# l90lpa/fv3-jedi-linearmodel

Hardware: AMD Instinct MI355X
Metric: column-updates/s per TL+AD dyn step (higher is better)
Workload: dtype f64; 1 GPU; C192L127 hydrostatic TL+AD, six cube faces dealt over 1 GPU(s) (6 per rank), table-driven exchange (221184 columns per GPU), k_split=2 n_split=6 dt=450s nq=4, hord mt/vt/tm/dp/tr=2/2/2/2/2 (sponge: 1/1/1/1 below level 9), kord=17, nord=1; columns_per_gpu=221184

## Files before the change

### fv3_jedi_linearmodel_amd/csrc/dycore.h

```cpp
#pragma once
#include "../../include/fv3lm.h"
#include "stages.h"
#include "column.h"
#include "exchange.h"
#include "nh.h"
#include "nh_ad.h"
#include "tpfused.h"
#include "tpad.h"
#include "tp2.h"
#include "dampt.h"
#include <functional>
#include <map>
#include <memory>
#include <set>
#include <string>
#include <vector>

namespace fv3 {

#ifdef FV3LM_HOST_EMUL
inline void* dev_alloc(size_t n) { void* p = std::calloc(n ? n : 1, 1); return p; }
inline void dev_free(void* p) { std::free(p); }
inline void dev_zero(Exec&, void* p, size_t n) { std::memset(p, 0, n); }
inline void dev_copy(Exec&, void* d, const void* s, size_t n) { std::memcpy(d, s, n); }
// ... 42 lines not shown
    Fld f; f.t = t + used; f.p = p + used; f.nk = nk; used += n; return f;
  }
};

struct CkSet {
  struct Item { std::string name; double* p; size_t n, off; };
  std::string name; std::vector<Item> items; size_t stride = 0; int nrec = 0; double* buf = nullptr;
  void add(const std::string& nm, double* p, size_t ndoubles) { items.push_back(Item{nm, p, ndoubles, stride}); stride += ndoubles; }
  void add(const std::string& nm, const Fld& f, size_t plane) { add(nm, f.t, (size_t)f.nk * plane); }
  void alloc(const char* nm, int nrec_) {
    name = nm; buf = nrec_ > 0 ? (double*)dev_alloc(stride * nrec_ * 8) : nullptr; nrec = buf ? nrec_ : 0;
    if (std::getenv("FV3LM_VERBOSE")) std::fprintf(stderr, "fv3lm: checkpoint set %s: %d records, %zu bytes\n", nm, nrec, stride * nrec * 8);
  }
  void destroy() { dev_free(buf); buf = nullptr; nrec = 0; }
  int item(const char* nm) const {
    for (int n = 0; n < (int)items.size(); ++n) if (items[(size_t)n].name == nm) return n;
    set_sticky("internal error: checkpoint set " + name + " has no item " + nm); return -1;
  }
  size_t bytes(int item) const { return items[(size_t)item].n * 8; }
  double* at(int rec, int item) const {
    if (buf && rec >= 0 && rec < nrec && item >= 0 && item < (int)items.size()) return buf + (size_t)rec * stride + items[(size_t)item].off;
    set_sticky("internal error: checkpoint set " + name + ": record " + std::to_string(rec) + " item " + std::to_string(item) + " out of range"); return nullptr;
  }
  void save(Exec& ex, int rec, int item) const { if (double* q_ = at(rec, item)) dev_copy(ex, q_, items[(size_t)item].p, bytes(item)); }
  void restore(Exec& ex, int rec, int item, double* to = nullptr) const {
    if (const double* q_ = at(rec, item)) dev_copy(ex, to ? to : items[(size_t)item].p, q_, bytes(item));
  }
  void save(Exec& ex, int rec) const { for (int n = 0; n < (int)items.size(); ++n) save(ex, rec, n); }
  void restore(Exec& ex, int rec) const { for (int n = 0; n < (int)items.size(); ++n) restore(ex, rec, n); }
  void redirect(Exec& ex, int rec, int item, const double* from) const { if (double* q_ = at(rec, item)) ex.redirect_t(from, q_); }
};

typedef fv3lm_options Options;

inline bool resolve_level(const Options& o, int k, int npz, LevelParams& lp) {
  int hord_m = o.hord_mt, hord_t = o.hord_tm, hord_v = o.hord_vt, hord_p = o.hord_dp;
  int nord_k = o.nord, nord_v = (2 > o.nord) ? o.nord : 2;
  double d2_divg = (0.20 > o.d2_bg) ? o.d2_bg : 0.20;
  double damp_vt = o.do_vort_damp ? o.vtdm4 : 0.;
  int nord_w = nord_v, nord_t = nord_v;
  double damp_w = damp_vt, damp_t = damp_vt, d_con_k = o.d_con;
  if (npz == 1 || o.n_sponge < 0) {
    d2_divg = o.d2_bg;
  } else if (k == 1) {
    nord_k = 0;
    if (0.01 < o.d2_bg) d2_divg = (o.d2_bg < o.d2_bg_k1) ? o.d2_bg_k1 : o.d2_bg;
    else if (0.01 < o.d2_bg_k1) d2_divg = o.d2_bg_k1;
    else d2_divg = 0.01;
    nord_w = 0; damp_w = d2_divg;
    if (o.do_vort_damp) { nord_v = 0; damp_vt = 0.5 * d2_divg; }
    d_con_k = 0.;
  } else {
    const int max1 = (2 < o.n_sponge - 1) ? o.n_sponge - 1 : 2;
    if (k == max1 && o.d2_bg_k2 > 0.01) {
      nord_k = 0; d2_divg = (o.d2_bg < o.d2_bg_k2) ? o.d2_bg_k2 : o.d2_bg;
      nord_w = 0; damp_w = d2_divg;
      if (o.do_vort_damp) { nord_v = 0; damp_vt = 0.5 * d2_divg; }
      d_con_k = 0.;
    } else {
      const int max2 = (3 < o.n_sponge) ? o.n_sponge : 3;
      if (k == max2 && o.d2_bg_k2 > 0.05) {
        nord_k = 0; d2_divg = (o.d2_bg < 0.2 * o.d2_bg_k2) ? 0.2 * o.d2_bg_k2 : o.d2_bg;
        nord_w = 0; damp_w = d2_divg; d_con_k = 0.;
      }
    }
  }
// ... 98 lines not shown
  bool reuse_fields = false;
  Fld S(const char* n, int nk) {
    if (reuse_fields) { auto it = F.find(n); if (it != F.end()) return it->second; }
    (nk == g.npz ? nS3 : nS3p)++; Fld x = state.take((size_t)ntile_all * nk * g.plane, nk); F[n] = x; return x; }
  int nW3 = 0, nW3p = 0, nS3 = 0, nS3p = 0;
  Fld W(const char* n, int nk) {
    if (reuse_fields) { auto it = F.find(n); if (it != F.end()) return it->second; }
    (nk == g.npz ? nW3 : nW3p)++; Fld x = work.take((size_t)ntile_all * nk * g.plane, nk); F[n] = x; return x; }

  Rect R(int i0, int i1, int j0, int j1) const { return Rect{i0, i1, j0, j1}; }
  static Rect empty_in(const Rect& r) { return Rect{r.i0 + 1, r.i0, r.j0 + 1, r.j0}; }
  static Rect isect(const Rect& a, const Rect& b) { return Rect{std::max(a.i0, b.i0), std::min(a.i1, b.i1), std::max(a.j0, b.j0), std::min(a.j1, b.j1)}; }
  static bool is_empty(const Rect& r) { return r.i0 > r.i1 || r.j0 > r.j1; }
  template <class D>
  void add_face(Program& P, const char* grp, const D& s, int W) {
    if (!g.face) { add(P, grp, Edged<D, false>(s)); return; }
    const int lo = 1 + W, hi = g.nx - W, BIG = 1 << 20;
    const Rect regs[5] = {{lo, hi, lo, hi}, {-BIG, BIG, -BIG, lo - 1}, {-BIG, BIG, hi + 1, BIG}, {-BIG, lo - 1, lo, hi}, {hi + 1, BIG, lo, hi}};
    std::vector<Edged<D, true>> strips; bool have_bulk = false; Edged<D, false> bulk;
    for (int r = 0; r < 5; ++r) {
      D t = s; Rect anchor{1, 0, 1, 0}; bool any = false;
      for (int n = 0; n < D::NOUT; ++n) {
        t.orect[n] = isect(s.orect[n], regs[r]);
        if (!is_empty(t.orect[n]) && !any) { anchor = t.orect[n]; any = true; }
      }
      if (!any) continue;
      for (int n = 0; n < D::NOUT; ++n) if (is_empty(t.orect[n])) t.orect[n] = empty_in(anchor);
      if (r == 0) {
        for (int m = 0; m < D::NIN; ++m) if ((edge_only_inputs((const D*)nullptr) >> m) & 1u) { const int nk = t.in[m].nk; t.in[m] = Fld{}; t.in[m].nk = nk; }
        bulk = Edged<D, false>(t); have_bulk = true;
      } else strips.push_back(Edged<D, true>(t));
    }
    const size_t n0 = P.size();
    add_multi(P, grp, strips);
    const size_t n1 = P.size();
    if (have_bulk) add(P, grp, bulk);
#ifndef FV3LM_HOST_EMUL
    if (have_bulk && n1 == n0 + 1 && P.size() == n1 + 1) {
      auto fs = P[n0].fn; auto fb = P[n1].fn;
      P[n0].fn = [fs](Exec& e, int mode) {
        if (mode == MODE_AD || !e.sstream) { fs(e, mode); return; }
        HIPCHK(hipEventRecord(e.ev_s0, e.stream)); HIPCHK(hipStreamWaitEvent(e.sstream, e.ev_s0, 0));
        hipStream_t main = e.stream; e.stream = e.sstream;
        fs(e, mode);
        e.stream = main;
        HIPCHK(hipEventRecord(e.ev_s1, e.sstream)); e.side_pending = true;
      };
      P[n1].fn = [fb](Exec& e, int mode) {
        fb(e, mode);
        if (e.side_pending) { HIPCHK(hipStreamWaitEvent(e.stream, e.ev_s1, 0)); e.side_pending = false; }
      };
    }
#endif
  }

  template <class St>
  static void declare(Op& op, const St& s) {
    for (int m = 0; m < St::NIN; ++m) if (St::wants(m) && s.in[m].p) { op.ad_in.push_back(s.in[m].p); op.ad_in_slot.push_back(m); }
    for (int n = 0; n < St::NOUT; ++n) { op.ad_out.push_back(s.out[n].p); op.ad_out_rect.push_back(s.orect[n]); }
  }
  template <class St>
  void add(Program& P, const char* group, const St& s) {
    Ctx* cp = &ctx;
    auto sp = std::make_shared<St>(s);
    Op op{group, [sp, cp](Exec& e, int mode) { run(e, mode, *sp, *cp); }};
    declare(op, s);
    op.set_wmask = [sp](unsigned w, Rect r) { sp->wmask = w; sp->wrect = r; };
    op.name = St::name();
    P.push_back(op);
  }
  template <class St>
  void add_multi(Program& P, const char* group, const std::vector<St>& v) {
    if (v.empty()) return;
    if (v.size() == 1) { add(P, group, v[0]); return; }
    Ctx* cp = &ctx;
    Op op{group, [v, cp](Exec& e, int mode) { run_multi(e, mode, v.data(), (int)v.size(), *cp); }};
    for (const St& s : v) declare(op, s);
    op.ad_in_slot.clear();
    op.name = St::name();
    P.push_back(op);
  }
  void halo(int mode, int kind, const Fld& f0, const Fld& f1 = Fld{}) {
    if (!g.face) { run_halo(ex, mode, g, f0); if (f1.t) run_halo(ex, mode, g, f1); return; }
    if (xt[kind].n == 0 && !xr[kind].active) { halo_missing = true; return; }
    run_exchange(ex, mode, g, xt[kind], ex.sh(f0), ex.sh(f1));
    if (!run_exchange_remote(ex, mode, g, xr[kind], ex.sh(f0), ex.sh(f1), err)) halo_missing = true;
  }
  void add_halo(Program& P, const char* group, int kind, Fld f0, Fld f1 = Fld{}, int when = 0) {
    Dycore* self = this;
    Op op{group, [self, kind, f0, f1, when](Exec&, int mode) {
      if (self->g.face && ((when == 1 && self->last_acoustic) || (when == 2 && !self->last_acoustic))) return;
      if (!self->g.face && when == 2) return;
      self->halo(mode, kind, f0, f1);
    }};
    op.ad_in = {f0.p, f1.p};
    op.name = "halo"; op.global = true;
    P.push_back(op);
  }
  void halo_window(int mode, bool start, int win, int kind, const Fld& f0, const Fld& f1) {
#ifndef FV3LM_HOST_EMUL
    if (ex.xstream) {
      if (start) {
        HIPCHK(hipEventRecord(ex.ev_a[win], ex.stream)); HIPCHK(hipStreamWaitEvent(ex.xstream, ex.ev_a[win], 0));
        hipStream_t main = ex.stream; ex.stream = ex.xstream;
        halo(mode, kind, f0, f1);
        ex.stream = main;
        HIPCHK(hipEventRecord(ex.ev_b[win], ex.xstream));
      } else HIPCHK(hipStreamWaitEvent(ex.stream, ex.ev_b[win], 0));
      return;
    }
#endif
    (void)win;
    if (!start) halo(mode, kind, f0, f1);
// ... 199 lines not shown
        }
        Op ad{grp, [a, cp, adf](Exec& e, int) { if (adf == 2) run_tp_ad(e, a, *cp); else run_tp_outer_ad(e, a, *cp); }};
        ad.modes = 1u << MODE_AD; ad.name = adf == 2 ? "TpAd" : "TpOuter";
        ad.ad_out = {fx.p, fy.p}; ad.ad_out_rect = {R(is, ie + 1, js, je), R(is, ie, js, je + 1)};
        if (adf == 2) ad.ad_in = {q.p, crx.p, cry.p, xfx.p, yfx.p, rax.p, ray.p, mx.p, my.p};
        else { ad.ad_store = {q_i.p, q_j.p, fx2.p, fy2.p}; ad.ad_in = {crx.p, cry.p, mx.p, my.p}; }
        P.push_back(ad);
      }
    }
  }
  void build_a2b(Program& P, const char* grp, const std::string& pre, Fld q, Fld qb, int nk) {
    const int is = g.is(), ie = g.ie(), js = g.js(), je = g.je();
    Fld qx = W((pre + "_qx").c_str(), nk), qy = W((pre + "_qy").c_str(), nk);
    const int npx = g.nx + 1, npy = g.ny + 1;
    A2bA_<false> a; a.in[0] = q; a.out[0] = qx; a.out[1] = qy; a.k1 = nk;
    A2bB_<false> b; b.in[0] = qx; b.in[1] = qy; b.in[2] = Fld{}; b.out[0] = qb; b.k1 = nk;
    if (!g.face) {
      a.orect[0] = R(is, ie + 1, js - 2, je + 2); a.orect[1] = R(is - 2, ie + 2, js, je + 1); add(P, grp, a);
      b.orect[0] = R(is, ie + 1, js, je + 1); add(P, grp, b);
      return;
    }
    const Rect qxr = R(is, ie + 1, std::max(1, js - 2), std::min(npy - 1, je + 2)), qyr = R(std::max(1, is - 2), std::min(npx - 1, ie + 2), js, je + 1);
    a.orect[0] = isect(qxr, R(3, npx - 2, qxr.j0, qxr.j1)); a.orect[1] = isect(qyr, R(qyr.i0, qyr.i1, 3, npy - 2));
    const bool a0 = !is_empty(a.orect[0]), a1 = !is_empty(a.orect[1]);
    if (a0 && !a1) a.orect[1] = empty_in(a.orect[0]);
    if (a1 && !a0) a.orect[0] = empty_in(a.orect[1]);
    A2bA_<true> ae; ae.in[0] = q; ae.out[0] = qx; ae.out[1] = qy; ae.k1 = nk;
    std::vector<A2bA_<true>> av;
    for (int e = 0; e < 4; ++e) {
      const Rect r = e == 0 ? isect(qxr, R(1, 2, qxr.j0, qxr.j1)) : e == 1 ? isect(qxr, R(npx - 1, npx, qxr.j0, qxr.j1)) : e == 2 ? isect(qyr, R(qyr.i0, qyr.i1, 1, 2)) : isect(qyr, R(qyr.i0, qyr.i1, npy - 1, npy));
      if (is_empty(r)) continue;
      ae.orect[e < 2 ? 0 : 1] = r; ae.orect[e < 2 ? 1 : 0] = empty_in(r); av.push_back(ae);
    }
    add_multi(P, grp, av);
    if (a0 || a1) add(P, grp, a);
    const Rect qbr = R(is, ie + 1, js, je + 1);
    b.orect[0] = isect(qbr, R(3, npx - 2, 3, npy - 2));
    A2bB_<true> be; be.in[0] = qx; be.in[1] = qy; be.in[2] = q; be.out[0] = qb; be.k1 = nk;
    std::vector<A2bB_<true>> bv;
    for (int e = 0; e < 4; ++e) {
      const Rect r = isect(qbr, e == 0 ? R(1, npx, 1, 2) : e == 1 ? R(1, npx, npy - 1, npy) : e == 2 ? R(1, 2, 3, npy - 2) : R(npx - 1, npx, 3, npy - 2));
      if (is_empty(r)) continue;
      be.orect[0] = r; bv.push_back(be);
    }
    add_multi(P, grp, bv);
    if (!is_empty(b.orect[0])) add(P, grp, b);
  }

  void build_acoustic();
  bool init(int nx, int ny, int npz, int ntile, int face, int nq_, double bdt_, int n_split_, int k_split_, const Options& o,
            const double* const* metrics_host, double da_min, double da_min_c, const double* phis_host, int nface = 0, const int* ij0 = nullptr);
  void destroy();

  void run_group(Progs& P, const char* group, int mode, bool skip_accum = false);
  void zero_work_adjoint() { dev_zero(ex, work.p, work.used * 8); }
  void dyn_core(int mode);
};

inline void Dycore::run_group(Progs& PS, const char* group, int mode, bool skip_accum) {
  const bool all = (group == nullptr) || (group[0] == 0);
  ex.skip_accum = skip_accum;
  const int nc = (int)PS.c.size();
  auto take = [&](const Op& op) { return (all || op.group == group) && !(mode != MODE_AD && skip_accum && op.accum) && ((op.modes >> mode) & 1u); };
  if (nc == 1) {
    set_class(0);
    const Program& P = PS.c[0];
    if (mode != MODE_AD) { for (const Op& op : P) if (take(op)) { if (op.global) set_class(-1); op.fn(ex, mode); if (op.global) set_class(0); } }
    else for (auto it = P.rbegin(); it != P.rend(); ++it) if (take(*it)) { if (it->global) set_class(-1); it->fn(ex, mode); if (it->global) set_class(0); }
    set_class(-1);
    ex.skip_accum = false;
    return;
  }
  std::vector<std::vector<size_t>> gl(nc);
  for (int c = 0; c < nc; ++c) for (size_t n = 0; n < PS.c[c].size(); ++n) if (PS.c[c][n].global) gl[c].push_back(n);
  for (int c = 1; c < nc; ++c) if (gl[c].size() != gl[0].size()) { set_sticky("internal error: the tile classes' programs hold different exchange sequences"); ex.skip_accum = false; return; }
  const size_t nseg = gl[0].size() + 1;
  auto seg = [&](int c, size_t sg, size_t& a, size_t& b) { a = sg == 0 ? 0 : gl[c][sg - 1] + 1; b = sg < gl[c].size() ? gl[c][sg] : PS.c[c].size(); };
  if (mode != MODE_AD) {
    for (size_t sg = 0; sg < nseg; ++sg) {
// ... 70 lines not shown
  if (!nh && npz < 2) { err = "hydrostatic vertical remap: the column map (edge values of cs_profile / scalar_profile) needs npz >= 2"; return false; }
  if (nh && !(o.a_imp > 0.5)) { err = "non-hydrostatic: a_imp must be > 0.5 (semi-implicit solver; the reference's a_imp <= 0.5 Riemann-invariant solver is not built)"; return false; }
  for (int kd : {o.kord_tm_pert, o.kord_mt_pert, o.kord_wz_pert, o.kord_tr_pert})
    if ((kd < 0 ? -kd : kd) <= 16) { err = "kord_*_pert: only |kord| > 16 (the linear profile, the one the TL/AD reference differentiates) is built"; return false; }
  for (int kd : {o.kord_tm, o.kord_mt, o.kord_wz, o.kord_tr}) {
    const int ak = kd < 0 ? -kd : kd;
    if (ak <= 16 && !(ak >= 8 && ak <= 15)) { err = "kord_tm/kord_mt/kord_wz/kord_tr: the linear profile (|kord| > 16) or, for the trajectory, the limited profiles 8 .. 15 of cs_profile / scalar_profile (not 16, not ppm_profile's 7 and below)"; return false; }
    if (ak <= 16 && npz < 6) { err = "kord: limited trajectory profiles need npz >= 6"; return false; }
  }
  lev_host.resize(npz + 1);
  for (int k = 1; k <= npz; ++k) {
    resolve_level(o, k, npz, lev_host[k - 1]);
    const LevelParams& l = lev_host[k - 1];
    for (int h : {l.hord_mt, l.hord_vt, l.hord_tm, l.hord_dp, l.hord_tr, l.hord_tm_g})
      if (h != 1 && h != 2 && h != 333) { err = "perturbation hord must be 1, 2 or 333 (the schemes the TL/AD reference implements)"; return false; }
    for (int h : {l.hord_mt_t, l.hord_vt_t, l.hord_tm_t, l.hord_dp_t, l.hord_tr_t, l.hord_tm_g_t})
      if (h != 333 && !(h >= 1 && h <= 13)) { err = "trajectory hord must be 1, 2, 333 (differentiated) or, with a different perturbation scheme, 3 .. 13"; return false; }
    const int pairs[6][2] = {{l.hord_mt_t, l.hord_mt}, {l.hord_vt_t, l.hord_vt}, {l.hord_tm_t, l.hord_tm}, {l.hord_dp_t, l.hord_dp}, {l.hord_tr_t, l.hord_tr}, {l.hord_tm_g_t, l.hord_tm_g}};
    for (auto& pr : pairs) if (pr[0] == pr[1] && pr[0] != 1 && pr[0] != 2 && pr[0] != 333) { err = "hord must be 1, 2 or 333 where trajectory and perturbation share the scheme"; return false; }
  }
#ifndef FV3LM_HOST_EMUL
  HIPCHK(hipStreamCreate(&ex.stream));
  { const char* env = std::getenv("FV3LM_NO_ASYNC_HALO");
    if (face && !(env && env[0] == '1')) {
      HIPCHK(hipStreamCreate(&ex.xstream));
      for (int w = 0; w < Exec::NWIN; ++w) { HIPCHK(hipEventCreateWithFlags(&ex.ev_a[w], hipEventDisableTiming)); HIPCHK(hipEventCreateWithFlags(&ex.ev_b[w], hipEventDisableTiming)); }
    }
    const char* es = std::getenv("FV3LM_NO_SIDE_STRIPS");
    if (face && !(es && es[0] == '1')) {
      HIPCHK(hipStreamCreate(&ex.sstream));
      HIPCHK(hipEventCreateWithFlags(&ex.ev_s0, hipEventDisableTiming)); HIPCHK(hipEventCreateWithFlags(&ex.ev_s1, hipEventDisableTiming));
    } }
#endif
  lev_host[npz] = lev_host[npz - 1];
  lev_dev = (LevelParams*)dev_alloc(sizeof(LevelParams) * (npz + 1));
  h2d(ex, lev_dev, lev_host.data(), sizeof(LevelParams) * (npz + 1));
  const size_t np = (size_t)ntile * g.plane;
  metric_dev.resize(NMETRIC);
  for (int m = 0; m < NMETRIC; ++m) { metric_dev[m] = (double*)dev_alloc(np * 8); h2d(ex, metric_dev[m], metrics_host[m], np * 8); }
  Metrics& M = ctx.m; int m = 0;
  const double** slots[] = {&M.area, &M.rarea, &M.rarea_c, &M.dx, &M.dy, &M.dxa, &M.dya, &M.dxc, &M.dyc, &M.rdx, &M.rdy, &M.rdxa,
                            &M.rdya, &M.rdxc, &M.rdyc, &M.cosa, &M.sina, &M.rsina, &M.cosa_u, &M.cosa_v, &M.cosa_s, &M.sina_u,
                            &M.sina_v, &M.rsin_u, &M.rsin_v, &M.rsin2, &M.f0, &M.fC, &M.del6_u, &M.del6_v, &M.divg_u, &M.divg_v};
  for (auto s : slots) *s = metric_dev[m++];
  M.sin_sg[0] = M.cos_sg[0] = nullptr;
  for (int n = 1; n <= 9; ++n) M.sin_sg[n] = metric_dev[m++];
  for (int n = 1; n <= 9; ++n) M.cos_sg[n] = metric_dev[m++];
  M.da_min = da_min; M.da_min_c = da_min_c;
  edge_dev = (double*)dev_alloc((size_t)ntile * 4 * g.pj * 8); ecorner_dev = (double*)dev_alloc((size_t)ntile * 12 * 8);
  M.edge = edge_dev; M.ecorner = ecorner_dev;
  m_all = M;
  hs_dev = (double*)dev_alloc(np * 8);
  if (phis_host) h2d(ex, hs_dev, phis_host, np * 8);
  ctx.g = g; ctx.lev = lev_dev; ctx.nlev = npz;
  n3 = np * npz; n3p = np * (npz + 1);
  state.init(n3 * (12 + (size_t)nq + (nh ? 5 + (size_t)nq : 0)) + n3p * (6 + (nh ? 2 : 0)) + np);
  if (nh) {
    nh_ws = (double*)dev_alloc((size_t)NH_WS_SLOTS * (npz + 2) * np * 8);
    const char* tape_env = std::getenv("FV3LM_NH_TAPE");
    const bool tape_on = tape_env && tape_env[0] == '1';
    nh_tape.cap = tape_on ? 104 * (npz + 2) : 1;
    int tape_tiles = tape_on ? ntile : 1;
    if (tape_on) {
#ifndef FV3LM_HOST_EMUL
    { size_t fr = 0, tot = 0;
      if (hipMemGetInfo(&fr, &tot) != hipSuccess) fr = 0;
// ... 170 lines not shown
    for (const char* n_ : {"w", "delz", "zh"}) st_in.push_back(n_);
    for (const char* n_ : {"w_o", "delz_o", "zh_o"}) st_out.push_back(n_);
  }
  Fld utmp = W("utmp", npz), vtmp = W("vtmp", npz), ua = W("ua", npz), va = W("va", npz);
  { CswInterpAD s; s.in[0] = u; s.in[1] = v; s.out[0] = utmp; s.out[1] = vtmp; s.out[2] = ua; s.out[3] = va;
    s.orect[0] = R(isd, ied, js - 1, je + 1); s.orect[1] = R(is - 1, ie + 1, jsd, jed);
    s.orect[2] = s.orect[3] = R(is - 1, ie + 1, js - 1, je + 1);
    if (g.face) {
      const int il = is == 1 ? isd : is - 1, ih = ie == g.nx ? ied : ie + 1, jl = js == 1 ? jsd : js - 1, jh = je == g.ny ? jed : je + 1;
      s.orect[0] = R(isd, ied, jl, jh); s.orect[1] = R(il, ih, jsd, jed); s.orect[2] = s.orect[3] = R(il, ih, jl, jh);
    }
    s.k1 = npz; add_face(P, "c_sw", s, 3); }
  Fld uc0 = W("uc0", npz), utf = W("utf", npz), vc0 = W("vc0", npz), vtf = W("vtf", npz);
  const Fld none{};
  { CswInterpC_<false> s; s.in[0] = utmp; s.in[1] = vtmp; s.in[2] = u; s.in[3] = v; s.out[0] = uc0; s.out[1] = utf; s.out[2] = vc0; s.out[3] = vtf;
    s.dt2 = dt2; s.k1 = npz;
    if (!g.face) {
      s.orect[0] = s.orect[1] = R(is - 1, ie + 2, js - 1, je + 1); s.orect[2] = s.orect[3] = R(is - 1, ie + 1, js - 1, je + 2); add(P, "c_sw", s);
    } else {
      const int npx = g.nx + 1, npy = g.ny + 1;
      const Rect ur = R(is - 1, ie + 2, js - 1, je + 1), vr = R(is - 1, ie + 1, js - 1, je + 2);
      s.orect[0] = s.orect[1] = isect(ur, R(3, npx - 2, ur.j0, ur.j1)); s.orect[2] = s.orect[3] = isect(vr, R(vr.i0, vr.i1, 3, npy - 2));
      const bool b0 = !is_empty(s.orect[0]), b2 = !is_empty(s.orect[2]);
      if (b0 && !b2) s.orect[2] = s.orect[3] = empty_in(s.orect[0]);
      if (b2 && !b0) s.orect[0] = s.orect[1] = empty_in(s.orect[2]);
      CswInterpC_<true> e; for (int n = 0; n < 4; ++n) { e.in[n] = s.in[n]; e.out[n] = s.out[n]; }
      e.in[4] = ua; e.in[5] = va; e.dt2 = dt2; e.k1 = npz;
      std::vector<CswInterpC_<true>> ev;
      for (int m = 0; m < 4; ++m) {
        const Rect r = m == 0 ? isect(ur, R(ur.i0, 2, ur.j0, ur.j1)) : m == 1 ? isect(ur, R(npx - 1, ur.i1, ur.j0, ur.j1)) : m == 2 ? isect(vr, R(vr.i0, vr.i1, vr.j0, 2)) : isect(vr, R(vr.i0, vr.i1, npy - 1, vr.j1));
        if (is_empty(r)) continue;
        e.orect[0] = e.orect[1] = m < 2 ? r : empty_in(r); e.orect[2] = e.orect[3] = m < 2 ? empty_in(r) : r; ev.push_back(e);
      }
      add_multi(P, "c_sw", ev);
      if (b0 || b2) add(P, "c_sw", s);
    } }
  Fld divgd = W("divgd", npz);
  if (opt.nord > 0) {
    CswDivgD s; s.in[0] = u; s.in[1] = v; s.in[2] = ua; s.in[3] = va; s.out[0] = divgd; s.orect[0] = R(is, ie + 1, js, je + 1); s.k1 = npz;
    add_face(P, "c_sw", s, 1);
  }
  Fld delpc = W("delpc", npz), ptc = W("ptc", npz);
  { CswTransportD s; s.in[0] = delp; s.in[1] = pt; s.in[2] = utf; s.in[3] = vtf; s.out[0] = delpc; s.out[1] = ptc;
    s.orect[0] = s.orect[1] = R(is - 1, ie + 1, js - 1, je + 1); s.k1 = npz; add_face(P, "c_sw", s, 1); }
  Fld wc{};
  if (nh) {
    wc = W("wc", npz);
    CswTransportWD s; s.in[0] = delp; s.in[1] = w; s.in[2] = utf; s.in[3] = vtf; s.in[4] = delpc; s.out[0] = wc;
    s.orect[0] = R(is - 1, ie + 1, js - 1, je + 1); s.k1 = npz; add_face(P, "c_sw", s, 1);
  }
  Fld ke_c = W("ke_c", npz), vort_c = W("vort_c", npz);
  { CswKeVortD s; s.in[0] = ua; s.in[1] = va; s.in[2] = uc0; s.in[3] = vc0; s.in[4] = g.face ? u : none; s.in[5] = g.face ? v : none; s.out[0] = ke_c; s.out[1] = vort_c;
    s.orect[0] = R(is - 1, ie + 1, js - 1, je + 1); s.orect[1] = R(is, ie + 1, js, je + 1); s.dt2 = dt2; s.k1 = npz; add_face(P, "c_sw", s, 1); }
  Fld uc1 = W("uc1", npz), vc1 = W("vc1", npz);
  { CswUpdateD s; s.in[0] = uc0; s.in[1] = vc0; s.in[2] = u; s.in[3] = v; s.in[4] = vort_c; s.in[5] = ke_c; s.out[0] = uc1; s.out[1] = vc1;
    s.orect[0] = R(is, ie + 1, js, je); s.orect[1] = R(is, ie, js, je + 1); s.dt2 = dt2; s.k1 = npz; add_face(P, "c_sw", s, 1); }
  Fld pe_c = W("pe_c", npz + 1), peln_c = W("peln_c", npz + 1), pkc = W("pkc", npz + 1), gz = W("gz", npz + 1);
  Fld uc = W("uc", npz), vc = W("vc", npz);
  if (nh) {
    Fld gz_a = W("gz_a", npz + 1);
    Fld xfz = W("xfz", npz + 1), yfz = W("yfz", npz + 1);
    { DzFluxC s; s.in[0] = utf; s.in[1] = vtf; s.out[0] = xfz; s.out[1] = yfz; s.orect[0] = R(is - 1, ie + 2, js - 1, je + 1);
      s.orect[1] = R(is - 1, ie + 1, js - 1, je + 2); s.k1 = npz + 1; add(P, "update_dz_c", s); }
    { UpdateDzCD s; s.in[0] = zh; s.in[1] = xfz; s.in[2] = yfz; s.out[0] = gz_a; s.orect[0] = R(is - 1, ie + 1, js - 1, je + 1); s.k1 = npz + 1;
      add_face(P, "update_dz_c", s, 1); }
    { NhColArgs a = nh_args(dt2); a.f[0] = gz_a; a.f[1] = wc; a.f[2] = ptc; a.f[3] = delpc; a.f[4] = gz; a.f[5] = pkc;
      add_col(P, "riem_c", NHC_RIEM_C, a, R(is - 1, ie + 1, js - 1, je + 1)); }
    PGradCNh s; s.in[0] = pkc; s.in[1] = gz; s.in[2] = uc1; s.in[3] = vc1; s.in[4] = delpc; s.out[0] = uc; s.out[1] = vc;
// ... 240 lines not shown
```

### fv3_jedi_linearmodel_amd/csrc/exec.h

```cpp
#pragma once
#include "core.h"
#include <cstddef>
#include <type_traits>
#include <string>
#include <vector>

namespace fv3 {

inline std::string& sticky_error() { static std::string e; return e; }
inline void set_sticky(const std::string& m) { if (sticky_error().empty()) sticky_error() = m; }

struct ProfRec { std::string name; double bytes; 
#ifndef FV3LM_HOST_EMUL
  hipEvent_t e0, e1;
#endif
};
struct Exec {
#ifndef FV3LM_HOST_EMUL
  hipStream_t stream = nullptr;
  hipStream_t xstream = nullptr;
  hipStream_t sstream = nullptr; hipEvent_t ev_s0 = nullptr, ev_s1 = nullptr; bool side_pending = false;
  static constexpr int NWIN = 4;
  hipEvent_t ev_a[NWIN] = {}, ev_b[NWIN] = {};
#endif
  bool check_boxes = false;
  bool skip_accum = false;
  bool no_wmask = false;
  double* wlo = nullptr; double* whi = nullptr; std::ptrdiff_t tshift = 0;
  size_t cls_off = 0;
  struct Redir { const double* from; double* to; };
  static constexpr int NREDIR = 24;
  Redir rt[NREDIR], rp[NREDIR]; int nrt = 0, nrp = 0;
  void redirect_t(const double* from, double* to) { if (nrt < NREDIR) rt[nrt++] = Redir{from, to}; else set_sticky("internal error: redirect table full"); }
  void redirect_p(const double* from, double* to) { if (nrp < NREDIR) rp[nrp++] = Redir{from, to}; else set_sticky("internal error: redirect table full"); }
  Fld sh(const Fld& f) const {
    Fld r = f;
    if (tshift && f.t >= wlo && f.t < whi) r.t = f.t + tshift;
    for (int k = 0; k < nrt; ++k) if (f.t == rt[k].from) { r.t = rt[k].to; break; }
    for (int k = 0; k < nrp; ++k) if (f.p == rp[k].from) { r.p = rp[k].to; break; }
    if (cls_off) { if (r.t) r.t += cls_off * (size_t)f.nk; if (r.p) r.p += cls_off * (size_t)f.nk; }
    return r;
  }
  long launches = 0;
  bool profiling = false;
  std::vector<ProfRec> recs;
  void mark_begin(const char* name, const char* suffix, double bytes) {
    if (!profiling) return;
    ProfRec r; r.name = std::string(name) + suffix; r.bytes = bytes;
#ifndef FV3LM_HOST_EMUL
    if (hipEventCreate(&r.e0) != hipSuccess || hipEventCreate(&r.e1) != hipSuccess || hipEventRecord(r.e0, stream) != hipSuccess) { set_sticky("profiling: hipEventCreate/Record failed"); profiling = false; return; }
#endif
    recs.push_back(r);
  }
  void mark_end() {
    if (!profiling) return;
#ifndef FV3LM_HOST_EMUL
    (void)hipEventRecord(recs.back().e1, stream);
// ... 220 lines not shown
struct AdLoop<S, M, true> {
  HD static void run(const S&, const Ctx&, const Rect&, int, int, int, int) {}
};
template <class S, class = void> struct hand_ad_of { static constexpr bool value = false; };
template <class S> struct hand_ad_of<S, typename std::enable_if<S::HAND_AD>::type> { static constexpr bool value = true; };
template <class S>
HD void ad_point(const S& s, const Ctx& c, const Rect& R, int i, int j, int z, int nkmax) {
  if constexpr (hand_ad_of<S>::value) { (void)nkmax; s.hand_ad(c, R, i, j, z); }
  else if constexpr (joint_ad((const S*)nullptr)) { body_ad_joint<S, 0>(s, c, R, i, j, z); body_ad_joint<S, 1>(s, c, R, i, j, z); }
  else AdLoop<S, 0>::run(s, c, R, i, j, z, nkmax);
}

template <class S>
inline Rect ad_input_rect(const S& s, const Ctx& c, const Rect& R) {
  Rect q = R;
  for (int m = 0; m < S::NIN; ++m) {
    Box b = S::box(m);
    if (R.i0 + b.di0 < q.i0) q.i0 = R.i0 + b.di0;
    if (R.i1 + b.di1 > q.i1) q.i1 = R.i1 + b.di1;
    if (R.j0 + b.dj0 < q.j0) q.j0 = R.j0 + b.dj0;
    if (R.j1 + b.dj1 > q.j1) q.j1 = R.j1 + b.dj1;
  }
  if (s.wmask && s.wrect.i0 <= s.wrect.i1) {
    if (s.wrect.i0 < q.i0) q.i0 = s.wrect.i0; if (s.wrect.i1 > q.i1) q.i1 = s.wrect.i1;
    if (s.wrect.j0 < q.j0) q.j0 = s.wrect.j0; if (s.wrect.j1 > q.j1) q.j1 = s.wrect.j1;
  }
  if (q.i0 < c.g.isd()) q.i0 = c.g.isd();
  if (q.j0 < c.g.jsd()) q.j0 = c.g.jsd();
  if (q.i1 > c.g.ied() + 1) q.i1 = c.g.ied() + 1;
  if (q.j1 > c.g.jed() + 1) q.j1 = c.g.jed() + 1;
  return q;
}

enum Mode { MODE_NL = 0, MODE_TL = 1, MODE_AD = 2 };
template <class S>
inline double stage_bytes(const S& s, const Ctx& c, const Rect& R, int mode) {
  const double cells = double(R.i1 - R.i0 + 1) * double(R.j1 - R.j0 + 1) * c.g.ntile * (s.k1 - s.k0 + 1);
  int nin = 0;
  for (int m = 0; m < S::NIN; ++m) if (s.in[m].t) nin++;
  const double per = mode == MODE_NL ? nin + S::NOUT : mode == MODE_TL ? 2. * (nin + S::NOUT) : (nin + S::NOUT + 2. * nin);
  return 8. * per * cells;
}

#ifndef FV3LM_HOST_EMUL
#ifndef FV3LM_BY
#define FV3LM_BY 4
#endif
constexpr int BX = 64, BY = FV3LM_BY;
#ifdef FV3LM_STAGE_WAVES
#define FV3LM_STAGE_ATTR __attribute__((amdgpu_waves_per_eu(FV3LM_STAGE_WAVES, 8)))
#else
#define FV3LM_STAGE_ATTR
#endif
HD void xcd_block(int gx, int gy, int& bx, int& by) {
  const int n = gx * gy, l = bx + gx * by, q = n / 8, r = n % 8, res = l % 8;
  const int logical = (res < r ? res * (q + 1) : r * (q + 1) + (res - r) * q) + l / 8;
  bx = logical % gx; by = logical / gx;
}
HD void thread_point(const Rect& R, int tr, int bx, int by, int tx, int ty, int& i, int& j) {
  if (tr) { const int rows = BX / tr; i = R.i0 + bx * tr + tx % tr; j = R.j0 + (by * BY + ty) * rows + tx / tr; }
  else { i = R.i0 + bx * BX + tx; j = R.j0 + by * BY + ty; }
}
template <class S>
__global__ void __launch_bounds__(BX* BY) FV3LM_STAGE_ATTR k_stage_nl(S s, Ctx c, Rect R, int tr) {
  int i, j, bx = blockIdx.x, by = blockIdx.y; xcd_block(gridDim.x, gridDim.y, bx, by); thread_point(R, tr, bx, by, threadIdx.x, threadIdx.y, i, j);
  if (i <= R.i1 && j <= R.j1) body_nl(s, c, i, j, blockIdx.z);
// ... 212 lines not shown
    }
}
template <class S, bool TL>
inline void launch_fw_lds(Exec& ex, const S& s, const Ctx& c, const Rect& R) {
  const int nz = c.g.ntile * (s.k1 - s.k0 + 1);
  const dim3 g((R.i1 - R.i0 + BX) / BX, (R.j1 - R.j0 + S::LDS_BY) / S::LDS_BY, (nz + LDS_NLEV - 1) / LDS_NLEV);
  hipLaunchKernelGGL((k_stage_fw_lds<S, TL>), g, dim3(BX, S::LDS_BY), TileLayout<S>::total * (TL ? 16 : 8) * LDS_NLEV, ex.stream, s, c, R, nz);
}
template <class S>
void run_nl(Exec& ex, const S& s, const Ctx& c) {
  Rect R = rect_union(s.orect, S::NOUT);
  ex.mark_begin(S::name(), ".nl", stage_bytes(s, c, R, MODE_NL));
  hipLaunchKernelGGL(k_stage_nl<S>, grid_for(R, c.g.ntile * (s.k1 - s.k0 + 1), strip_tr(R)), dim3(BX, BY), 0, ex.stream, s, c, R, strip_tr(R));
  ex.mark_end();
  ex.launches++;
}
template <class S>
void run_tl(Exec& ex, const S& s, const Ctx& c) {
  Rect R = rect_union(s.orect, S::NOUT);
  ex.mark_begin(S::name(), ".tl", stage_bytes(s, c, R, MODE_TL));
  if constexpr (lds_fw<S>::value) if constexpr (TileLayout<S>::total > 0 && TileLayout<S>::total * 16 <= 60000) { if (strip_tr(R) == 0) {
    launch_fw_lds<S, true>(ex, s, c, R);
    ex.mark_end(); ex.launches++; return; } }
  hipLaunchKernelGGL(k_stage_tl<S>, grid_for(R, c.g.ntile * (s.k1 - s.k0 + 1), strip_tr(R)), dim3(BX, BY), 0, ex.stream, s, c, R, strip_tr(R));
  ex.mark_end();
  ex.launches++;
}
template <class S>
void run_ad(Exec& ex, const S& s, const Ctx& c) {
  Rect R = rect_union(s.orect, S::NOUT);
  Rect Q = ad_input_rect(s, c, R);
  int nkmax = 0;
  for (int m = 0; m < S::NIN; ++m) if (s.in[m].nk > nkmax) nkmax = s.in[m].nk;
  ex.mark_begin(S::name(), ".ad", stage_bytes(s, c, R, MODE_AD));
  if constexpr (lds_ad<S>::value) if constexpr (TileLayoutAd<S>::ok() && TileLayoutAd<S>::total * 8 <= 60000) { if (strip_tr(Q) == 0) {
    bool same = true;
    for (int m = 0; m < S::NIN; ++m) if (s.in[m].nk != s.in[0].nk) same = false;
    if (same) {
      const dim3 gq((Q.i1 - Q.i0 + BX) / BX, (Q.j1 - Q.j0 + S::LDS_BY) / S::LDS_BY, c.g.ntile * s.in[0].nk);
      hipLaunchKernelGGL(k_stage_ad_lds<S>, gq, dim3(BX, S::LDS_BY), TileLayoutAd<S>::total * 8, ex.stream, s, c, R, Q);
      ex.mark_end(); ex.launches++; return; } } }
  hipLaunchKernelGGL(k_stage_ad<S>, grid_for(Q, c.g.ntile * nkmax, strip_tr(Q)), dim3(BX, BY), 0, ex.stream, s, c, R, Q, nkmax, strip_tr(Q));
  ex.mark_end();
  ex.launches++;
  if constexpr (S::NALIAS > 0) if (c.g.face) {
    ex.mark_begin(S::name(), ".ad_corner", 0.);
    hipLaunchKernelGGL(k_stage_ad_alias<S>, dim3(4, c.g.ntile * nkmax), dim3(64), 0, ex.stream, s, c, R);
    ex.mark_end();
    ex.launches++;
  }
}
constexpr int MAXSTRIP = 4;
template <class S>
struct Multi { S s[MAXSTRIP]; Rect R[MAXSTRIP]; int n, boff[MAXSTRIP + 1], gx[MAXSTRIP], tr[MAXSTRIP]; };
template <class S, bool TL>
__global__ void __launch_bounds__(BX* BY) k_stage_multi_fw(Multi<S> m, Ctx c) {
  int b = blockIdx.x, r = 0;
  while (r + 1 < m.n && b >= m.boff[r + 1]) ++r;
  b -= m.boff[r];
  int i, j; thread_point(m.R[r], m.tr[r], b % m.gx[r], b / m.gx[r], threadIdx.x, threadIdx.y, i, j);
  if (i > m.R[r].i1 || j > m.R[r].j1) return;
  if (TL) body_tl(m.s[r], c, i, j, blockIdx.z); else body_nl(m.s[r], c, i, j, blockIdx.z);
}
template <class S>
__global__ void __launch_bounds__(BX* BY) k_stage_multi_ad(Multi<S> m, Rect Q0, Rect Q1, Rect Q2, Rect Q3, Ctx c, int nkmax) {
  const Rect Q[MAXSTRIP] = {Q0, Q1, Q2, Q3};
  int b = blockIdx.x, r = 0;
  while (r + 1 < m.n && b >= m.boff[r + 1]) ++r;
  b -= m.boff[r];
  int i, j; thread_point(Q[r], m.tr[r], b % m.gx[r], b / m.gx[r], threadIdx.x, threadIdx.y, i, j);
  if (i > Q[r].i1 || j > Q[r].j1) return;
  for (int r2 = 0; r2 < r; ++r2) if (Q[r2].has(i, j)) return;
  if (0 >= r && 0 < m.n && Q0.has(i, j)) ad_point(m.s[0], c, m.R[0], i, j, blockIdx.z, nkmax);
  if (1 >= r && 1 < m.n && Q1.has(i, j)) ad_point(m.s[1], c, m.R[1], i, j, blockIdx.z, nkmax);
  if (2 >= r && 2 < m.n && Q2.has(i, j)) ad_point(m.s[2], c, m.R[2], i, j, blockIdx.z, nkmax);
  if (3 >= r && 3 < m.n && Q3.has(i, j)) ad_point(m.s[3], c, m.R[3], i, j, blockIdx.z, nkmax);
}
// ... 111 lines not shown
  ex.launches++;
}
#else
template <class S>
void run_nl(Exec& ex, const S& s, const Ctx& c) {
  Rect R = rect_union(s.orect, S::NOUT);
  for (int z = 0; z < c.g.ntile * (s.k1 - s.k0 + 1); ++z)
    for (int j = R.j0; j <= R.j1; ++j)
      for (int i = R.i0; i <= R.i1; ++i) body_nl(s, c, i, j, z);
  ex.launches++;
}
template <class S>
void run_tl(Exec& ex, const S& s, const Ctx& c) {
  Rect R = rect_union(s.orect, S::NOUT);
  const int nl = s.k1 - s.k0 + 1;
  for (int z = 0; z < c.g.ntile * nl; ++z)
    for (int j = R.j0; j <= R.j1; ++j)
      for (int i = R.i0; i <= R.i1; ++i) {
        if (ex.check_boxes) {
          Dual o[S::NOUT];
          AccChk<S> a{s, c, z / nl, s.k0 + z % nl, i, j};
          s.template eval<Dual>(a, c, z / nl, i, j, s.k0 + z % nl, o);
        }
        body_tl(s, c, i, j, z);
      }
  ex.launches++;
}
template <class S>
void run_ad(Exec& ex, const S& s, const Ctx& c) {
  Rect R = rect_union(s.orect, S::NOUT);
  Rect Q = ad_input_rect(s, c, R);
  int nkmax = 0;
  for (int m = 0; m < S::NIN; ++m) if (s.in[m].nk > nkmax) nkmax = s.in[m].nk;
  for (int z = 0; z < c.g.ntile * nkmax; ++z)
    for (int j = Q.j0; j <= Q.j1; ++j)
      for (int i = Q.i0; i <= Q.i1; ++i) ad_point(s, c, R, i, j, z, nkmax);
  if constexpr (S::NALIAS > 0) if (c.g.face)
    for (int z = 0; z < c.g.ntile * nkmax; ++z)
      for (int cn = 0; cn < 4; ++cn)
        for (int n = 0; n < 4 * c.g.ng * c.g.ng; ++n) {
          int i, j;
          corner_block_point(c.g, cn, n, i, j);
          if (!c.g.in_plane(i, j)) continue;
          AdAliasLoop<S, 0>::run(s, c, R, i, j, z);
        }
  ex.launches++;
}
template <class F>
void for_points(Exec& ex, const Rect& R, int nz, const F& f, const char* tag = "points", double bytes = 0.) {
  for (int z = 0; z < nz; ++z)
    for (int j = R.j0; j <= R.j1; ++j)
      for (int i = R.i0; i <= R.i1; ++i) f(i, j, z);
  ex.launches++;
}
#endif

template <class S>
void run(Exec& ex, int mode, const S& s0, const Ctx& c);
#ifdef FV3LM_HOST_EMUL
template <class S>
void run_multi(Exec& ex, int mode, const S* s0, int n, const Ctx& c) { for (int r = 0; r < n; ++r) run(ex, mode, s0[r], c); }
#endif
template <class S>
void run(Exec& ex, int mode, const S& s0, const Ctx& c) {
  S s = s0;
  if (ex.no_wmask) s.wmask = 0;
  for (int m = 0; m < S::NIN; ++m) s.in[m] = ex.sh(s.in[m]);
  for (int n = 0; n < S::NOUT; ++n) s.out[n] = ex.sh(s.out[n]);
  if (mode == MODE_NL) run_nl(ex, s, c);
  else if (mode == MODE_TL) run_tl(ex, s, c);
  else run_ad(ex, s, c);
}

}
```

Baseline: 183,800 column-updates/s.

## Overlap adjoint edge-strip stages with bulk interior on a side stream

In adjoint mode, stages split into a bulk kernel plus edge strips now have the bulk adjoint divided into an inner rectangle that does not touch the strips' input footprints and a set of frame bands. The frame bands and strip adjoints run on the side stream while the inner part runs concurrently on the main stream, joined by an event. The goal is to hide the serialized strip launches behind bulk work in the AD sweep. The cost is extra launches and planning, and by default a long list of stages is excluded through a skip list. Correctness relies on the disjointness checks and on rejecting in/out pointer aliasing.

```diff
diff --git a/fv3_jedi_linearmodel_amd/csrc/dycore.h b/fv3_jedi_linearmodel_amd/csrc/dycore.h
--- a/fv3_jedi_linearmodel_amd/csrc/dycore.h
+++ b/fv3_jedi_linearmodel_amd/csrc/dycore.h
@@ -98,6 +98,7 @@
 };
 
 typedef fv3lm_options Options;
+constexpr const char* AD_SIDE_SKIP_DEFAULT = "CswDivg,CswInterpA,CswKeVort,CswTransport,CswUpdate,DdB,DswKe,DswWindsA,TpD2,CswTransportW,UpdateDzC";
 
 inline bool resolve_level(const Options& o, int k, int npz, LevelParams& lp) {
   int hord_m = o.hord_mt, hord_t = o.hord_tm, hord_v = o.hord_vt, hord_p = o.hord_dp;
@@ -262,9 +263,10 @@
       } else strips.push_back(Edged<D, true>(t));
     }
     const size_t n0 = P.size();
-    add_multi(P, grp, strips);
+    auto es = add_multi(P, grp, strips);
     const size_t n1 = P.size();
-    if (have_bulk) add(P, grp, bulk);
+    std::shared_ptr<Edged<D, false>> bs;
+    if (have_bulk) bs = add(P, grp, bulk);
 #ifndef FV3LM_HOST_EMUL
     if (have_bulk && n1 == n0 + 1 && P.size() == n1 + 1) {
       auto fs = P[n0].fn; auto fb = P[n1].fn;
@@ -282,6 +284,7 @@
       };
     }
 #endif
+    side_ad(P, n0, n1, bs, es);
   }
 
   template <class St>
@@ -290,7 +293,7 @@
     for (int n = 0; n < St::NOUT; ++n) { op.ad_out.push_back(s.out[n].p); op.ad_out_rect.push_back(s.orect[n]); }
   }
   template <class St>
-  void add(Program& P, const char* group, const St& s) {
+  std::shared_ptr<St> add(Program& P, const char* group, const St& s) {
     Ctx* cp = &ctx;
     auto sp = std::make_shared<St>(s);
     Op op{group, [sp, cp](Exec& e, int mode) { run(e, mode, *sp, *cp); }};
@@ -298,17 +301,68 @@
     op.set_wmask = [sp](unsigned w, Rect r) { sp->wmask = w; sp->wrect = r; };
     op.name = St::name();
     P.push_back(op);
+    return sp;
   }
   template <class St>
-  void add_multi(Program& P, const char* group, const std::vector<St>& v) {
-    if (v.empty()) return;
-    if (v.size() == 1) { add(P, group, v[0]); return; }
+  std::vector<std::shared_ptr<St>> add_multi(Program& P, const char* group, const std::vector<St>& v) {
+    if (v.empty()) return {};
+    if (v.size() == 1) return {add(P, group, v[0])};
     Ctx* cp = &ctx;
-    Op op{group, [v, cp](Exec& e, int mode) { run_multi(e, mode, v.data(), (int)v.size(), *cp); }};
+    auto vp = std::make_shared<std::vector<St>>(v);
+    Op op{group, [vp, cp](Exec& e, int mode) { run_multi(e, mode, vp->data(), (int)vp->size(), *cp); }};
     for (const St& s : v) declare(op, s);
     op.ad_in_slot.clear();
     op.name = St::name();
     P.push_back(op);
+    std::vector<std::shared_ptr<St>> out;
+    for (St& s : *vp) out.push_back(std::shared_ptr<St>(vp, &s));
+    return out;
+  }
+  template <class B, class E>
+  void side_ad(Program& P, size_t n0, size_t n1, std::shared_ptr<B> b, const std::vector<std::shared_ptr<E>>& ev) {
+    if (!b || ev.empty() || n1 != n0 + 1 || P.size() != n1 + 1 || B::NALIAS > 0) return;
+    Ctx* cp = &ctx;
+    auto fs = P[n0].fn; auto fb = P[n1].fn;
+    auto done = std::make_shared<bool>(false);
+    auto listed = std::make_shared<bool>(false);
+    const std::string key = std::string(",") + B::name() + ",";
+    P[n1].fn = [=](Exec& e, int mode) {
+      *done = false;
+      AdSplit sp;
+      std::vector<const E*> es; for (auto& q_ : ev) es.push_back(q_.get());
+      bool split = mode == MODE_AD && e.side_ad && e.n_ad_part == 0 && e.ad_side_skip.find(key) == std::string::npos;
+#ifndef FV3LM_HOST_EMUL
+      split = split && e.sstream;
+#endif
+      const bool planned = split && plan_side_ad(e, *cp, *b, es, sp);
+      if (mode == MODE_AD && e.ad_side_list && !*listed) {
+        *listed = true;
+        std::fprintf(stderr, "side_ad %s: %s", B::name(), planned ? "split" : "in line");
+        if (planned) std::fprintf(stderr, ", inner %d..%d x %d..%d, %d frame bands", sp.inner.i0, sp.inner.i1, sp.inner.j0, sp.inner.j1, sp.nframe);
+        std::fprintf(stderr, "\n");
+      }
+      if (!planned) { fb(e, mode); return; }
+      auto part = [&](const Rect* r, int n, const char* tag) { for (int k = 0; k < n; ++k) e.ad_part[k] = r[k]; e.n_ad_part = n; e.ad_tag = tag; fb(e, mode); e.n_ad_part = 0; e.ad_tag = ".ad"; };
+#ifndef FV3LM_HOST_EMUL
+      HIPCHK(hipEventRecord(e.ev_s0, e.stream)); HIPCHK(hipStreamWaitEvent(e.sstream, e.ev_s0, 0));
+      hipStream_t main = e.stream; e.stream = e.sstream;
+      if (sp.nframe) part(sp.frame, sp.nframe, ".ad_frame");
+      fs(e, mode);
+      e.stream = main;
+      HIPCHK(hipEventRecord(e.ev_s1, e.sstream));
+      part(&sp.inner, 1, ".ad");
+      HIPCHK(hipStreamWaitEvent(e.stream, e.ev_s1, 0));
+#else
+      part(&sp.inner, 1, ".ad");
+      if (sp.nframe) part(sp.frame, sp.nframe, ".ad_frame");
+      fs(e, mode);
+#endif
+      *done = true;
+    };
+    P[n0].fn = [=](Exec& e, int mode) {
+      if (mode == MODE_AD && *done) { *done = false; return; }
+      fs(e, mode);
+    };
   }
   void halo(int mode, int kind, const Fld& f0, const Fld& f1 = Fld{}) {
     if (!g.face) { run_halo(ex, mode, g, f0); if (f1.t) run_halo(ex, mode, g, f1); return; }
@@ -574,8 +628,10 @@
       if (is_empty(r)) continue;
       ae.orect[e < 2 ? 0 : 1] = r; ae.orect[e < 2 ? 1 : 0] = empty_in(r); av.push_back(ae);
     }
-    add_multi(P, grp, av);
-    if (a0 || a1) add(P, grp, a);
+    const size_t na0 = P.size();
+    auto aes = add_multi(P, grp, av);
+    const size_t na1 = P.size();
+    if (a0 || a1) side_ad(P, na0, na1, add(P, grp, a), aes);
     const Rect qbr = R(is, ie + 1, js, je + 1);
     b.orect[0] = isect(qbr, R(3, npx - 2, 3, npy - 2));
     A2bB_<true> be; be.in[0] = qx; be.in[1] = qy; be.in[2] = q; be.out[0] = qb; be.k1 = nk;
@@ -585,8 +641,10 @@
       if (is_empty(r)) continue;
       be.orect[0] = r; bv.push_back(be);
     }
-    add_multi(P, grp, bv);
-    if (!is_empty(b.orect[0])) add(P, grp, b);
+    const size_t nb0 = P.size();
+    auto bes = add_multi(P, grp, bv);
+    const size_t nb1 = P.size();
+    if (!is_empty(b.orect[0])) side_ad(P, nb0, nb1, add(P, grp, b), bes);
   }
 
   void build_acoustic();
@@ -723,6 +781,10 @@
       HIPCHK(hipEventCreateWithFlags(&ex.ev_s0, hipEventDisableTiming)); HIPCHK(hipEventCreateWithFlags(&ex.ev_s1, hipEventDisableTiming));
     } }
 #endif
+  {
+    const char* en = std::getenv("FV3LM_NO_SIDE_AD_STRIPS"); const char* sk = std::getenv("FV3LM_AD_SIDE_SKIP");
+    ex.side_ad = face && !(en && en[0] == '1'); ex.ad_side_list = std::getenv("FV3LM_AD_SIDE_LIST") != nullptr;
+    ex.ad_side_skip = "," + std::string(sk ? sk : AD_SIDE_SKIP_DEFAULT) + ","; }
   lev_host[npz] = lev_host[npz - 1];
   lev_dev = (LevelParams*)dev_alloc(sizeof(LevelParams) * (npz + 1));
   h2d(ex, lev_dev, lev_host.data(), sizeof(LevelParams) * (npz + 1));
@@ -959,8 +1021,10 @@
         if (is_empty(r)) continue;
         e.orect[0] = e.orect[1] = m < 2 ? r : empty_in(r); e.orect[2] = e.orect[3] = m < 2 ? empty_in(r) : r; ev.push_back(e);
       }
-      add_multi(P, "c_sw", ev);
-      if (b0 || b2) add(P, "c_sw", s);
+      const size_t n0 = P.size();
+      auto es = add_multi(P, "c_sw", ev);
+      const size_t n1 = P.size();
+      if (b0 || b2) side_ad(P, n0, n1, add(P, "c_sw", s), es);
     } }
   Fld divgd = W("divgd", npz);
   if (opt.nord > 0) {
diff --git a/fv3_jedi_linearmodel_amd/csrc/exec.h b/fv3_jedi_linearmodel_amd/csrc/exec.h
--- a/fv3_jedi_linearmodel_amd/csrc/exec.h
+++ b/fv3_jedi_linearmodel_amd/csrc/exec.h
@@ -23,6 +23,8 @@
   static constexpr int NWIN = 4;
   hipEvent_t ev_a[NWIN] = {}, ev_b[NWIN] = {};
 #endif
+  bool side_ad = false, ad_side_list = false; std::string ad_side_skip;
+  Rect ad_part[4] = {}; int n_ad_part = 0; const char* ad_tag = ".ad";
   bool check_boxes = false;
   bool skip_accum = false;
   bool no_wmask = false;
@@ -309,6 +311,45 @@
   return q;
 }
 
+struct AdSplit { Rect inner{1, 0, 1, 0}; Rect frame[4] = {}; int nframe = 0; };
+inline bool rects_meet(const Rect& a, const Rect& b) { return !(a.i1 < b.i0 || b.i1 < a.i0 || a.j1 < b.j0 || b.j1 < a.j0); }
+inline double rect_points(const Rect& r) { return (r.i0 > r.i1 || r.j0 > r.j1) ? 0. : double(r.i1 - r.i0 + 1) * double(r.j1 - r.j0 + 1); }
+inline bool ad_split_ok(const Rect& Q, const Rect* w, int nw, const AdSplit& sp) {
+  double pts = rect_points(sp.inner);
+  if (pts <= 0. || sp.inner.i0 < Q.i0 || sp.inner.i1 > Q.i1 || sp.inner.j0 < Q.j0 || sp.inner.j1 > Q.j1) return false;
+  for (int n = 0; n < nw; ++n) if (rect_points(w[n]) > 0. && rects_meet(w[n], sp.inner)) return false;
+  for (int f = 0; f < sp.nframe; ++f) {
+    const Rect& r = sp.frame[f];
+    if (rect_points(r) <= 0. || r.i0 < Q.i0 || r.i1 > Q.i1 || r.j0 < Q.j0 || r.j1 > Q.j1 || rects_meet(r, sp.inner)) return false;
+    for (int f2 = 0; f2 < f; ++f2) if (rects_meet(r, sp.frame[f2])) return false;
+    pts += rect_points(r);
+  }
+  return pts == rect_points(Q);
+}
+inline bool ad_split(const Rect& Q, const Rect* w, int nw, AdSplit& sp) {
+  Rect in = Q;
+  for (int n = 0; n < nw; ++n) {
+    const Rect& r = w[n];
+    if (rect_points(r) <= 0. || !rects_meet(r, in)) continue;
+    const double wd = in.i1 - in.i0 + 1, ht = in.j1 - in.j0 + 1;
+    const double cost[4] = {(r.j1 + 1 - in.j0) * wd, (in.j1 - (r.j0 - 1)) * wd, (r.i1 + 1 - in.i0) * ht, (in.i1 - (r.i0 - 1)) * ht};
+    int best = 0;
+    for (int k = 1; k < 4; ++k) if (cost[k] < cost[best]) best = k;
+    if (best == 0) in.j0 = r.j1 + 1; else if (best == 1) in.j1 = r.j0 - 1; else if (best == 2) in.i0 = r.i1 + 1; else in.i1 = r.i0 - 1;
+    if (in.i0 > in.i1 || in.j0 > in.j1) return false;
+  }
+  sp.inner = in; sp.nframe = 0;
+  if (in.j0 > Q.j0) sp.frame[sp.nframe++] = Rect{Q.i0, Q.i1, Q.j0, in.j0 - 1};
+  if (in.j1 < Q.j1) sp.frame[sp.nframe++] = Rect{Q.i0, Q.i1, in.j1 + 1, Q.j1};
+  if (in.i0 > Q.i0) sp.frame[sp.nframe++] = Rect{Q.i0, in.i0 - 1, in.j0, in.j1};
+  if (in.i1 < Q.i1) sp.frame[sp.nframe++] = Rect{in.i1 + 1, Q.i1, in.j0, in.j1};
+  const bool ok = ad_split_ok(Q, w, nw, sp);
+#ifdef FV3LM_HOST_EMUL
+  if (!ok) { std::fprintf(stderr, "ad_split: inner (%d..%d, %d..%d) and %d frame bands do not partition (%d..%d, %d..%d) clear of the strips\n", in.i0, in.i1, in.j0, in.j1, sp.nframe, Q.i0, Q.i1, Q.j0, Q.j1); std::abort(); }
+#endif
+  return ok;
+}
+
 enum Mode { MODE_NL = 0, MODE_TL = 1, MODE_AD = 2 };
 template <class S>
 inline double stage_bytes(const S& s, const Ctx& c, const Rect& R, int mode) {
@@ -587,17 +628,26 @@
   Rect Q = ad_input_rect(s, c, R);
   int nkmax = 0;
   for (int m = 0; m < S::NIN; ++m) if (s.in[m].nk > nkmax) nkmax = s.in[m].nk;
-  ex.mark_begin(S::name(), ".ad", stage_bytes(s, c, R, MODE_AD));
+  const int npart = ex.n_ad_part ? ex.n_ad_part : 1;
+  const double bytes = stage_bytes(s, c, R, MODE_AD), qpts = double(Q.i1 - Q.i0 + 1) * double(Q.j1 - Q.j0 + 1);
+  bool lds = false;
   if constexpr (lds_ad<S>::value) if constexpr (TileLayoutAd<S>::ok() && TileLayoutAd<S>::total * 8 <= 60000) { if (strip_tr(Q) == 0) {
-    bool same = true;
-    for (int m = 0; m < S::NIN; ++m) if (s.in[m].nk != s.in[0].nk) same = false;
-    if (same) {
-      const dim3 gq((Q.i1 - Q.i0 + BX) / BX, (Q.j1 - Q.j0 + S::LDS_BY) / S::LDS_BY, c.g.ntile * s.in[0].nk);
-      hipLaunchKernelGGL(k_stage_ad_lds<S>, gq, dim3(BX, S::LDS_BY), TileLayoutAd<S>::total * 8, ex.stream, s, c, R, Q);
-      ex.mark_end(); ex.launches++; return; } } }
-  hipLaunchKernelGGL(k_stage_ad<S>, grid_for(Q, c.g.ntile * nkmax, strip_tr(Q)), dim3(BX, BY), 0, ex.stream, s, c, R, Q, nkmax, strip_tr(Q));
-  ex.mark_end();
-  ex.launches++;
+    lds = true;
+    for (int m = 0; m < S::NIN; ++m) if (s.in[m].nk != s.in[0].nk) lds = false; } }
+  for (int p = 0; p < npart; ++p) {
+    const Rect P = ex.n_ad_part ? ex.ad_part[p] : Q;
+    if (P.i0 < Q.i0 || P.i1 > Q.i1 || P.j0 < Q.j0 || P.j1 > Q.j1 || P.i0 > P.i1 || P.j0 > P.j1) { set_sticky("internal error: adjoint part outside the launch rectangle"); return; }
+    ex.mark_begin(S::name(), ex.ad_tag, bytes * (double(P.i1 - P.i0 + 1) * double(P.j1 - P.j0 + 1) / qpts));
+    bool launched = false;
+    if constexpr (lds_ad<S>::value) if constexpr (TileLayoutAd<S>::ok() && TileLayoutAd<S>::total * 8 <= 60000) if (lds) {
+      const dim3 gq((P.i1 - P.i0 + BX) / BX, (P.j1 - P.j0 + S::LDS_BY) / S::LDS_BY, c.g.ntile * s.in[0].nk);
+      hipLaunchKernelGGL(k_stage_ad_lds<S>, gq, dim3(BX, S::LDS_BY), TileLayoutAd<S>::total * 8, ex.stream, s, c, R, P);
+      launched = true; }
+    if (!launched) hipLaunchKernelGGL(k_stage_ad<S>, grid_for(P, c.g.ntile * nkmax, strip_tr(P)), dim3(BX, BY), 0, ex.stream, s, c, R, P, nkmax, strip_tr(P));
+    ex.mark_end();
+    ex.launches++;
+  }
+  if (lds || ex.n_ad_part) return;
   if constexpr (S::NALIAS > 0) if (c.g.face) {
     ex.mark_begin(S::name(), ".ad_corner", 0.);
     hipLaunchKernelGGL(k_stage_ad_alias<S>, dim3(4, c.g.ntile * nkmax), dim3(64), 0, ex.stream, s, c, R);
@@ -775,9 +825,15 @@
   Rect Q = ad_input_rect(s, c, R);
   int nkmax = 0;
   for (int m = 0; m < S::NIN; ++m) if (s.in[m].nk > nkmax) nkmax = s.in[m].nk;
-  for (int z = 0; z < c.g.ntile * nkmax; ++z)
-    for (int j = Q.j0; j <= Q.j1; ++j)
-      for (int i = Q.i0; i <= Q.i1; ++i) ad_point(s, c, R, i, j, z, nkmax);
+  const int npart = ex.n_ad_part ? ex.n_ad_part : 1;
+  for (int p = 0; p < npart; ++p) {
+    const Rect P = ex.n_ad_part ? ex.ad_part[p] : Q;
+    if (P.i0 < Q.i0 || P.i1 > Q.i1 || P.j0 < Q.j0 || P.j1 > Q.j1 || P.i0 > P.i1 || P.j0 > P.j1) { std::fprintf(stderr, "stage %s: adjoint part outside the launch rectangle\n", S::name()); std::abort(); }
+    for (int z = 0; z < c.g.ntile * nkmax; ++z)
+      for (int j = P.j0; j <= P.j1; ++j)
+        for (int i = P.i0; i <= P.i1; ++i) ad_point(s, c, R, i, j, z, nkmax);
+  }
+  if (ex.n_ad_part) { ex.launches += npart; return; }
   if constexpr (S::NALIAS > 0) if (c.g.face)
     for (int z = 0; z < c.g.ntile * nkmax; ++z)
       for (int cn = 0; cn < 4; ++cn)
@@ -815,4 +871,39 @@
   else run_ad(ex, s, c);
 }
 
-}
+template <class S>
+inline S resolved(const Exec& ex, const S& s0) {
+  S s = s0;
+  if (ex.no_wmask) s.wmask = 0;
+  for (int m = 0; m < S::NIN; ++m) s.in[m] = ex.sh(s.in[m]);
+  for (int n = 0; n < S::NOUT; ++n) s.out[n] = ex.sh(s.out[n]);
+  return s;
+}
+template <class B, class E>
+inline bool plan_side_ad(const Exec& ex, const Ctx& c, const B& b0, const std::vector<const E*>& ev, AdSplit& sp) {
+  if (ev.empty() || ev.size() > 4) return false;
+  const B b = resolved(ex, b0);
+  const Rect Qb = ad_input_rect(b, c, rect_union(b.orect, B::NOUT));
+  Rect w[8]; int nw = 0;
+  const double* ins[(B::NIN + 4 * E::NIN)]; const double* outs[(B::NOUT + 4 * E::NOUT)]; int ni = 0, no = 0;
+  for (int m = 0; m < B::NIN; ++m) if (b.in[m].p) ins[ni++] = b.in[m].p;
+  for (int n = 0; n < B::NOUT; ++n) if (b.out[n].p) outs[no++] = b.out[n].p;
+  for (const E* e0 : ev) {
+    const E e = resolved(ex, *e0);
+    w[nw++] = ad_input_rect(e, c, rect_union(e.orect, E::NOUT));
+    for (int m = 0; m < E::NIN; ++m) if (e.in[m].p) ins[ni++] = e.in[m].p;
+    for (int n = 0; n < E::NOUT; ++n) if (e.out[n].p) outs[no++] = e.out[n].p;
+  }
+  if (E::NALIAS > 0 && c.g.face)
+    for (int cn = 0; cn < 4; ++cn) {
+      int i0, j0; corner_block_point(c.g, cn, 0, i0, j0);
+      Rect r{i0, i0 + 2 * c.g.ng - 1, j0, j0 + 2 * c.g.ng - 1};
+      if (r.i0 < c.g.isd()) r.i0 = c.g.isd(); if (r.i1 > c.g.ied() + 1) r.i1 = c.g.ied() + 1;
+      if (r.j0 < c.g.jsd()) r.j0 = c.g.jsd(); if (r.j1 > c.g.jed() + 1) r.j1 = c.g.jed() + 1;
+      w[nw++] = r;
+    }
+  for (int a = 0; a < ni; ++a) for (int o = 0; o < no; ++o) if (ins[a] == outs[o]) return false;
+  return ad_split(Qb, w, nw, sp);
+}
+
+}
```

Measured after the change: 184,600 column-updates/s (median of 6 runs). Within noise of the previous version (+0.4%).
